# HugoVuach/Dense-linear-app

Hardware: AMD Instinct MI355X
Metric: fp64 TFLOP/s for NxN SPD Cholesky (N^3/3 flops / factorisation time) (higher is better)
Workload: dtype f64

## Files before the change

dense_linear_app_amd/_lib.py:

```python
from __future__ import annotations

import ctypes as C
import os

_HERE = os.path.dirname(os.path.abspath(__file__))
LIB_PATH = os.environ.get("LIBCHOLMI_PATH") or os.path.join(_HERE, "libcholmi.so")

_lib = None


class CholmiError(RuntimeError):

    def __init__(self, fn: str, code: int, msg: str):
        super().__init__(f"{fn} failed with status {code}: {msg}")
        self.fn, self.code, self.msg = fn, code, msg


def lib() -> C.CDLL:
    global _lib
    if _lib is not None:
        return _lib
    if not os.path.exists(LIB_PATH):
        raise ImportError(
            f"{LIB_PATH} is missing: build it with `python -c 'import __graft_entry__ as g; g.build()'` "
# ... 19 lines not shown
        "chol_plgsy_tile": ([d, i, vp, u64], i),
        "chol_lacpy_tile": ([i, vp, vp], i),
        "chol_lange_tile": ([i, vp, C.POINTER(d)], i),
        "chol_lauum_tile": ([i, vp], i),
        "chol_geadd_tile": ([i, d, vp, d, vp], i),
        "chol_potrs_tile": ([i, vp, vp], i),
        "chol_posv_tile": ([i, vp, vp], i),
        "chol_dsposv_tile": ([i, vp, vp, vp, C.POINTER(i)], i),
        "chol_last_dsposv_stats": ([C.POINTER(d)], i),
        "chol_trtri_tile": ([i, i, vp], i),
        "chol_potri_tile": ([i, vp], i),
        "chol_poinv_tile": ([i, vp], i),
        "chol_lansy_tile": ([i, i, vp, C.POINTER(d)], i),
        "chol_pocon_tile": ([i, vp, d, C.POINTER(d)], i),
        "chol_last_pocon_stats": ([C.POINTER(d)], i),
        "chol_poequ_tile": ([vp, vp, C.POINTER(d), C.POINTER(d)], i),
        "chol_laqsy_tile": ([i, vp, vp, d, d, C.POINTER(i)], i),
        "chol_porfs_tile": ([i, vp, vp, vp, vp, C.POINTER(d), C.POINTER(d)], i),
        "chol_posvx_tile": ([i, i, vp, vp, C.POINTER(i), vp, vp, vp, C.POINTER(d), C.POINTER(d), C.POINTER(d)], i),
        "chol_last_posvx_stats": ([C.POINTER(d)], i),
        "chol_bench_refine": ([i, vp, vp, vp, i, i, C.POINTER(d)], i),
        "chol_pstrf_tile": ([i, vp, C.POINTER(i), C.POINTER(i), d], i),
        "chol_last_pstrf_stats": ([C.POINTER(d)], i),
        "chol_sygst_tile": ([i, i, vp, vp], i),
        "chol_last_sygst_stats": ([C.POINTER(d)], i),
        "chol_chud_tile": ([i, vp, vp], i),
        "chol_chdd_tile": ([i, vp, vp], i),
        "chol_last_chud_stats": ([C.POINTER(d)], i),
        "chol_trtrs_tile": ([i, i, i, vp, vp], i),
        "chol_trmm_tile": ([i, i, i, i, d, vp, vp], i),
        "chol_logdet_tile": ([vp, C.POINTER(d)], i),
        "chol_last_trtrs_stats": ([C.POINTER(d)], i),
        "chol_debug_half_limits": ([i, i], i),
        "chol_sytrf_nopiv_tile": ([i, vp], i),
        "chol_sytrs_nopiv_tile": ([i, vp, vp], i),
        "chol_sysv_nopiv_tile": ([i, vp, vp], i),
        "chol_last_sytrf_stats": ([C.POINTER(d)], i),
        "chol_rbt_apply_tile": ([i, vp, vp, i], i),
        "chol_sytrf_rbt_tile": ([i, vp, vp, i, u64], i),
        "chol_sytrs_rbt_tile": ([i, vp, vp, i, vp], i),
        "chol_sysv_rbt_tile": ([i, vp, vp, vp, i, u64, vp, vp, C.POINTER(i), C.POINTER(d)], i),
        "chol_last_rbt_stats": ([C.POINTER(d)], i),
        "chol_lapack_to_tile": ([vp, i, vp], i),
        "chol_tile_to_lapack": ([vp, vp, i], i),
        "chol_tile_upload": ([vp, i, i, vp], i),
        "chol_tile_download": ([vp, i, i, vp], i),
        "chol_residual_plgsy": ([vp, d, u64, C.POINTER(d)], i),
        "chol_residual_plgsy_inf": ([vp, d, u64, C.POINTER(d)], i),
        "chol_make_spd_like_chameleon": ([vp, i, i, d, C.c_char, u64], None),
        "chol_enforce_strict_diag_dominance": ([vp, i, i, d], None),
        "chol_extract_block": ([vp, i, i, i, i, i, vp], None),
        "chol_parse_payloads": ([C.c_char_p, vp, i, vp, vp, vp, vp], i),
        "chol_debug_flow_waves": ([], i),
        "chol_last_potrf_regimes": ([C.POINTER(i), C.POINTER(i)], i),
        "chol_debug_schedule_check": ([i, i, d, d, i, C.c_char_p, i], i),
        "chol_debug_schedule_check_grid": ([i, i, i, i, i, d, d, i, C.c_char_p, i], i),
        "chol_debug_comm_trace": ([i, i, i, i, i, d, d, C.c_char_p, i], i),
        "chol_debug_task_record": ([i, i], i),
        "chol_debug_task_check": ([C.POINTER(C.c_longlong)], i),
        "chol_last_potrf_stats": ([C.POINTER(d), C.POINTER(d), C.POINTER(i), C.POINTER(d)], i),
        "chol_set_profiling": ([i], i),
        "chol_debug_stamps": ([i, C.POINTER(C.c_ulonglong), i], i),
        "chol_mfma_probe": ([i, i, C.POINTER(d)], i),
        "chol_bench_update": ([vp, i, i, i, C.POINTER(d), C.POINTER(d)], i),
        "chol_desc_local_ptr": ([vp, C.POINTER(C.c_size_t)], vp),
        "chol_desc_local_tiles": ([vp, C.POINTER(i), C.POINTER(i)], i),
        "chol_set_transport": ([vp], i),
        "chol_transport_rccl_unique_id": ([vp], i),
        "chol_transport_rccl_init": ([vp, i, i], i),
        "chol_transport_rccl_finalize": ([], i),
        "chol_transport_rccl_version": ([], i),
        "chol_set_transport_channel": ([i, vp], i),
        "chol_transport_selftest": ([i, C.c_size_t], i),
        "chol_set_transport_null": ([], i),
        "chol_dist_rehearse": ([i, i, i, i, i, d, u64, vp, C.POINTER(d)], i),
        "chol_desc_set_version": ([vp, u64], i),
        "chol_tile_batch": ([i, i, i, i, vp, vp, vp, vp, vp, i], i),
        "chol_sync": ([], i),
        "chol_potrf_batch": ([i, i, i, vp, vp, vp, C.POINTER(i), i], i),
        "chol_batch_info": ([i, C.POINTER(i)], i),
        "chol_batch_stats": ([C.POINTER(C.c_longlong)], i),
        "chol_batch_mark": ([C.POINTER(C.c_ulonglong)], i),
        "chol_batch_wait": ([C.POINTER(C.c_ulonglong)], i),
        "chol_debug_calibration": ([C.POINTER(d)], i),
        "chol_debug_update_kernel": ([i, C.c_char_p, i], i),
        "chol_debug_device_counters": ([], i),
        "chol_dist_last_stats": ([C.POINTER(d), C.POINTER(C.c_longlong), C.POINTER(C.c_longlong), C.POINTER(C.c_longlong)], i),
        "chol_dist_factorize_with": ([vp, vp, i, i, i, i, i, i], i),
        "chol_dist_gather_lower": ([vp, vp, i], i),
    }
    for name, (argt, rest) in sig.items():
        try:
            fn = getattr(L, name)
        except AttributeError:
            if os.environ.get("LIBCHOLMI_PATH"):
                continue
            raise
        fn.argtypes = argt
        fn.restype = rest
    _lib = L
    return L


ABI_SYMBOLS = None


# ... 14 lines not shown
```

dense_linear_app_amd/csrc/api.hip:

```cpp
#include <hip/hip_runtime.h>

#include <algorithm>
#include <array>
#include <cmath>
#include <cstdarg>
#include <cstdio>
#include <cstdlib>
#include <cstring>
#include <deque>
#include <mutex>
#include <string>
#include <unordered_map>
#include <vector>

#include "../../include/cholmi.h"
#include "api_internal.h"
#include "cholmi_internal.h"

using namespace cholmi;

extern "C" int chol_internal_walk(chol_desc *d, void *base, cholmi::RankCtx *r, int rank);
extern "C" void chol_internal_dist_finalize(void);
extern "C" int chol_internal_desc_create(chol_desc_t **desc, void *mat, int dtype, int mb, int nb, int bsiz, int lm, int ln,
                                         int i, int j, int m, int n, int p, int q, int my_rank, int nranks);
// ... 789 lines not shown
  }
  for (hipStream_t s : r->retired) (void)hipStreamDestroy(s);
  r->retired.clear();
}

}

extern "C" {

int chol_internal_fail(int code, const char *msg) { return fail(code, msg); }

const char *chol_version(void) { return "cholmi 0.3 (gfx950)"; }

const char *chol_last_error(void) {
  static thread_local std::string copy;
  std::lock_guard<std::mutex> lk(g_err_mu);
  copy = g.last_error;
  return copy.c_str();
}

int chol_set_device(int device) {
  std::lock_guard<std::recursive_mutex> lk(g_mu);
  if (g.inited && device != g.r.device) return fail(-1, "chol_set_device after chol_init");
  g.r.device = device;
  return 0;
}

int chol_set_rank(int rank, int nranks) {
  if (nranks < 1 || rank < 0 || rank >= nranks) return fail(-1, "chol_set_rank: bad rank");
  g.rank = rank;
  g.nranks = nranks;
  return 0;
}

int chol_init(int ncpu, int ngpu) {
  (void)ncpu;
  std::lock_guard<std::recursive_mutex> lk(g_mu);
  if (g.inited) return 0;
  if (ngpu < 1)
    return fail(CHOL_ERR_NO_GPU, "chol_init: ngpu must be >= 1 (this library has no CPU backend)");
  int count = 0;
  hipError_t e = hipGetDeviceCount(&count);
  if (e != hipSuccess || count < 1) {
    (void)hipGetLastError();
    return fail(CHOL_ERR_NO_GPU, "chol_init: no HIP device visible");
  }
  if (g.r.device < 0) {
    const char *lr = getenv("LOCAL_RANK");
    g.r.device = lr ? atoi(lr) % count : 0;
  }
  if (g.r.device >= count) return fail(CHOL_ERR_NO_GPU, "chol_init: device index out of range");
  HIPCHECK(hipSetDevice(g.r.device));
  if (const char *e = getenv("CHOLMI_TRSM_SMALL_MAX")) cholmi::g_trsm_small_max = atoi(e);
  {
    hipDeviceProp_t prop;
    HIPCHECK(hipGetDeviceProperties(&prop, g.r.device));
    const int room = (prop.multiProcessorCount - 32) / 4;
    cholmi::g_poll_max_wgs = room < 0 ? 0 : (room < 48 ? room : 48);
  }
  if (const char *e = getenv("CHOLMI_POLL_MAX_WGS")) cholmi::g_poll_max_wgs = atoi(e);
  if (const char *e = getenv("CHOLMI_FLOW")) cholmi::g_flow = atoi(e);
  if (const char *e = getenv("CHOLMI_FLOW_NBM")) {
    int lo = 0, hi = 0;
    if (sscanf(e, "%d:%d", &lo, &hi) == 2) cholmi::g_flow_min_nbm = std::max(2, lo), cholmi::g_flow_max_nbm = std::min(8, hi);
  }
  if (const char *e = getenv("CHOLMI_FLOW_FENCES")) cholmi::g_flow_fences = atoi(e);
  if (const char *e = getenv("CHOLMI_INTILE_FUSED")) cholmi::g_intile_fused = atoi(e);
  if (const char *e = getenv("CHOLMI_MIN_UNITS")) cholmi::g_min_units = atoi(e);
  HIPCHECK(hipMalloc(&g.d_acc, 2 * sizeof(double)));
  HIPCHECK(hipMalloc(&g.d_ytab, YTAB_ENTRIES * sizeof(int)));
  HIPCHECK(hipMemset(g.d_ytab, 0, YTAB_ENTRIES * sizeof(int)));
  cholmi::g_ytab = g.d_ytab;
  int rc = rank_ctx_create(&g.r, g.r.device, nullptr);
  if (rc) return rc;
  g.inited = true;
  return 0;
}

int chol_finalize(void) {
  std::lock_guard<std::recursive_mutex> lk(g_mu);
  if (!g.inited) return 0;
  (void)hipDeviceSynchronize();
  chol_internal_dist_finalize();
  g.stage.release();
  g.work.release();
  spd_release();
  if (g.wc_winv) (void)hipFree(g.wc_winv);
  g.wc_winv = nullptr;
  if (g.d_binfo) (void)hipFree(g.d_binfo);
  g.d_binfo = nullptr;
  tx_destroy();
  g.wc_ptr = nullptr;
  g.wc_version = 0;
  (void)hipFree(g.d_acc);
  if (g.d_ytab) (void)hipFree(g.d_ytab);
  g.d_ytab = nullptr;
  cholmi::g_ytab = nullptr;
  rank_ctx_destroy(&g.r);
  g.d_acc = nullptr;
  g.inited = false;
  return 0;
}

int chol_desc_create(chol_desc_t **desc, void *mat, int dtype, int mb, int nb, int bsiz, int lm,
                     int ln, int i, int j, int m, int n, int p, int q) {
  return chol_internal_desc_create(desc, mat, dtype, mb, nb, bsiz, lm, ln, i, j, m, n, p, q, g.rank, g.nranks);
// ... 818 lines not shown
    HIPCHECK(hipEventRecord(g.r.events[1], g.r.st[ST_MAIN]));
    HIPCHECK(hipStreamSynchronize(g.r.st[ST_MAIN]));
    float t = 0;
    HIPCHECK(hipEventElapsedTime(&t, g.r.events[0], g.r.events[1]));
    if (r > 0 && t < best) best = t;
  }
  *ms = best;
  const double ntl = (double)(d->nt - 1 - k);
  if (flops) *flops = (ntl * (ntl - 1) + ntl) * (double)d->mbi * d->mbi * d->mbi;
  return 0;
}

int chol_debug_stamps(int enable, unsigned long long *out, int max_pairs) {
  if (!g.inited) return fail(CHOL_ERR_NOT_INITIALIZED, "debug_stamps before chol_init");
  static unsigned long long *buf = nullptr;
  const size_t bytes = (1 + 8 * 1000) * sizeof(unsigned long long);
  HIPCHECK(hipDeviceSynchronize());
  if (enable) {
    if (!buf) HIPCHECK(hipMalloc(&buf, bytes));
    HIPCHECK(hipMemset(buf, 0, bytes));
    cholmi::g_dbg = buf;
    return 0;
  }
  int n = 0;
  if (buf && out) {
    std::vector<unsigned long long> h(1 + 8 * 1000);
    HIPCHECK(hipMemcpy(h.data(), buf, bytes, hipMemcpyDeviceToHost));
    n = (int)std::min<unsigned long long>(h[0], (unsigned long long)std::min(max_pairs, 1000));
    memcpy(out, h.data() + 1, (size_t)n * 8 * sizeof(unsigned long long));
  }
  cholmi::g_dbg = nullptr;
  return n;
}

int chol_mfma_probe(int dtype, int waves_per_simd, double *tflops) {
  if (!g.inited) return fail(CHOL_ERR_NOT_INITIALIZED, "mfma_probe before chol_init");
  if (!tflops || waves_per_simd < 1 || waves_per_simd > 8) return fail(-2, "mfma_probe: arguments");
  std::lock_guard<std::recursive_mutex> lk(g_mu);
  return mfma_probe_on(&g.r, dtype, waves_per_simd, 4000, tflops);
}

int chol_debug_device_counters(void) { return g.inited && g.r.d_sem ? 1 : 0; }

int chol_debug_update_kernel(int dtype, char *buf, int buflen) {
  if (!buf || buflen < 8) return fail(-2, "debug_update_kernel: buffer");
  const bool f64 = dtype == CHOL_REAL_DOUBLE;
  if (!f64 && dtype != CHOL_REAL_FLOAT) return fail(-1, "debug_update_kernel: dtype");
  snprintf(buf, buflen, f64 ? "cholmi::k_trail_update_w8<double, 3>" : "cholmi::k_trail_update_w8f");
  return 0;
}

int chol_debug_flow_waves(void) { return g.r.flow_waves; }

int chol_last_potrf_regimes(int *out8, int *nt) {
  if (!out8) return fail(-1, "last_potrf_regimes: NULL");
  for (int i = 0; i < 8; ++i) out8[i] = g.r.regimes[i];
  if (nt) *nt = g.r.regimes_nt;
  return 0;
}

int chol_debug_calibration(double *out8) {
  if (!g.inited) return fail(CHOL_ERR_NOT_INITIALIZED, "debug_calibration before chol_init");
  if (!out8) return fail(-1, "debug_calibration: NULL");
  for (int i = 0; i < 2; ++i) {
    out8[2 * i] = g.r.probe_tflops[i];
    out8[2 * i + 1] = g.r.diag_us[i];
    out8[4 + 2 * i] = g.r.probe_tflops[i] * CHOLMI_UPDATE_EFF;
    out8[5 + 2 * i] = g.r.diag_us[i] * CHOLMI_STEP_FACTOR;
  }
  return 0;
}

}
```

dense_linear_app_amd/csrc/cholmi_internal.h:

```cpp
#pragma once
#include <hip/hip_runtime.h>
#include <stdint.h>
#include <algorithm>
#include <vector>

#include "../../include/cholmi.h"

struct chol_desc {
  int dtype, mb, nb, bsiz, lm, ln, i, j, m, n, p, q;
  int mbi, bsizi;
  bool padded;
  int mt, nt;
  int prow, pcol;
  int lmt, lnt;
  size_t esize;
  void *mat;
  bool on_device;
  bool owns;
  int2 *d_list = nullptr;
  std::vector<int> ge, gd;
  int n_off = 0;
  unsigned long long version = 0;
  void *user_mat = nullptr;
  int user_lmt = 0;
// ... 31 lines not shown
  }
  void free_all();
};

struct RankCtx {
  int device = -1;
  hipStream_t st[ST_COUNT] = {};
  void *winv = nullptr;
  size_t winv_bytes = 0;
  int *d_info = nullptr;
  int *d_sem = nullptr;
  bool flow_ok = false;
  unsigned tile_sem_next = 0;
  std::vector<hipEvent_t> events;
  std::vector<hipStream_t> retired;
  int stream_swaps = 0;
  int stream_collisions = 0;
  hipEvent_t ev_flow = nullptr;
  bool profiling = false;
  double total_ms = 0, update_ms = 0, update_flops = 0, issue_us = 0;
  int update_launches = 0;
  int flow_waves = 0;
  int regimes[8] = {};
  int regimes_nt = 0;
  long long sends = 0, recvs = 0, bytes_sent = 0;
  DevPool pool;
  double probe_tflops[2] = {0, 0}, diag_us[2] = {0, 0};
};
int rank_ctx_create(RankCtx *r, int device, const RankCtx *calib_from);
void rank_ctx_destroy(RankCtx *r);
RankCtx *main_rank_ctx();
int main_rank(int *nranks);

constexpr double CHOLMI_UPDATE_EFF = 0.85, CHOLMI_STEP_FACTOR = 2.65;

constexpr int MACRO = 128;
constexpr int MAXP = 8;

struct PanelRef {
  const void *base[MAXP];
  int first[MAXP];
  int P;
};

struct LocalMat {
  void *base;
  int lmt;
  int P, Q;
  int mb;
  long bsiz;
};

extern int g_trsm_small_max;
extern int g_poll_max_wgs;
bool flow_applies(int nbm);
extern int g_flow;
extern int g_flow_min_nbm;
extern int g_flow_max_nbm;
extern int g_flow_fences;
extern int g_intile_fused;
extern int g_min_units;
extern unsigned long long *g_dbg;
extern int *g_ytab;
constexpr int YTAB_ENTRIES = 2048;

template <typename T>
void launch_trail_update(hipStream_t s, const LocalMat &C, const int2 *d_list, int off, int na, int offb,
                         int nb, const PanelRef &pan, bool yield = false, const PanelRef *pan2 = nullptr);

template <typename T>
void launch_syr2k_update(hipStream_t s, const LocalMat &C, const int2 *d_list, int off, int na, int offb, int nb,
                         const PanelRef &pan, const PanelRef &qan);

template <typename T>
void launch_ldl_update(hipStream_t s, const LocalMat &C, const int2 *d_list, int off, int na, int offb, int nb,
                       const PanelRef &pan, const PanelRef &qan);

template <typename T>
void launch_potrf_tile(hipStream_t s, T *tile, int mb, T *winv, int *d_info, int info_base, int *sem = nullptr);

template <typename T>
void launch_diag_syrk(hipStream_t s, T *C, const T *A, int mb);

void launch_sem_probe(hipStream_t consumer, hipStream_t producer, int *sem, int *result);
void launch_pipe_probe(hipStream_t big, hipStream_t small, unsigned long long *t, int cus);

struct SyrkPipe {
  void *c;
  hipStream_t su;
  int *sem;
  int *fc = nullptr;
  hipStream_t sflow = nullptr;
  hipEvent_t ev_flow = nullptr;
  bool join_flow = false;
};
inline int flow_ctl_lines(int nbm) { return nbm >= 2 && nbm <= 8 ? 1 + nbm + 2 * nbm * nbm : 0; }

template <typename T>
void launch_panel_pipelined(hipStream_t sp, hipStream_t st, hipEvent_t *ev, T *lkk, int mb, T *winv,
                            int *d_info, int info_base, T *tiles, long bsiz, int ntiles,
                            hipEvent_t ev_head = nullptr, const SyrkPipe *sy = nullptr, const int *wait_sem = nullptr,
                            int wait_target = 0, int *tile_sem = nullptr);

template <typename T>
void launch_col_update_small(hipStream_t s, T *C, const T *A, const T *B, int mb, int ntiles, long bsiz, int *done);

// ... 211 lines not shown
```

dense_linear_app_amd/csrc/kernels.hip:

```cpp
#include "cholmi_internal.h"
#include "mfma_traits.h"

#include <type_traits>

#if defined(__HIP_DEVICE_COMPILE__) && !defined(__gfx950__)
#error "libcholmi's kernels target gfx950 (MI355X) only: build with --offload-arch=gfx950"
#endif

namespace cholmi {

constexpr int BK = 16;
constexpr int LROW = MACRO + 16;

template <int I, int N, typename F>
__device__ __forceinline__ void static_for(F &&f) {
  if constexpr (I < N) {
    f(std::integral_constant<int, I>{});
    static_for<I + 1, N>(f);
  }
}


template <typename T>
struct alignas(16) Smem {
// ... 776 lines not shown
  update_ptr_block<CoreW8<T, MODE>>(cin, ap, bp, cout, n, mb, nbm, unit, ytab, sm);
}
__global__ __launch_bounds__(512, 4) void k_update_ptrs_w8f(const float *const *__restrict__ cin, const float *const *__restrict__ ap,
                                                             const float *const *__restrict__ bp, float *const *__restrict__ cout,
                                                             int n, int mb, int nbm, int unit, const int *ytab) {
  __shared__ SmemF sm;
  update_ptr_block<CoreW8F>(cin, ap, bp, cout, n, mb, nbm, unit, ytab, sm);
}

template <typename T>
__global__ __launch_bounds__(256, 2) void k_panel_solve(T *tiles, long bsiz, int mb, int nbm,
                                                        int s, const T *__restrict__ winv, T alpha,
                                                        int *ytab, const int *wait_sem = nullptr,
                                                        int wait_target = 0, int *fail = nullptr,
                                                        int *head_sem = nullptr) {
  __shared__ SmemP<T> sm;
  sem_wait(wait_sem, wait_target, fail);
  GuestOnCu guest(ytab);
  __builtin_amdgcn_s_setprio(2);
  const int tix = blockIdx.x / nbm, r = blockIdx.x % nbm;
  T *Ap = tiles + (long)tix * bsiz + r * MACRO + (long)s * MACRO * mb;
  const T *Bp = winv + (long)s * MACRO * MACRO;
  Acc<T> acc;
  acc_zero<T>(acc);
  nt_kloop_paired<T>(Ap, mb, Bp, MACRO, MACRO, acc, sm);
  nt_epilogue_paired<T>(Ap, mb, acc, alpha, T(0), false);
  guest.leave();
  if (tix == 0) sem_signal(head_sem);
}

template <typename T>
__global__ __launch_bounds__(256, 2) void k_panel_update(T *tiles, long bsiz, int mb, int nbm, int s,
                                                         const T *__restrict__ lkk, T beta, int *ytab,
                                                         const int *wait_sem = nullptr, int wait_target = 0,
                                                         int *fail = nullptr) {
  __shared__ SmemP<T> sm;
  sem_wait(wait_sem, wait_target, fail);
  GuestOnCu guest(ytab);
  __builtin_amdgcn_s_setprio(2);
  const int nc = nbm - 1 - s;
  int b = blockIdx.x;
  const int c = s + 1 + b % nc;
  b /= nc;
  const int r = b % nbm, tix = b / nbm;
  T *tile = tiles + (long)tix * bsiz;
  const T *Ap = tile + r * MACRO + (long)s * MACRO * mb;
  const T *Bp = lkk + c * MACRO + (long)s * MACRO * mb;
  T *Cp = tile + r * MACRO + (long)c * MACRO * mb;
  Acc<T> acc;
  acc_zero<T>(acc);
  nt_kloop_paired<T>(Ap, mb, Bp, mb, MACRO, acc, sm);
  nt_epilogue_paired<T>(Cp, mb, acc, T(-1), beta, false);
  guest.leave();
}

constexpr int SK = 32;
template <typename T, int ROWS>
struct SmallImg {
  T v[SK][ROWS + 16];
};
template <typename T, int ROWS>
__device__ __forceinline__ void small_gload(const T *__restrict__ P, int ld, int k0, T (&r)[ROWS * SK / 256]) {
#pragma unroll
  for (int q = 0; q < ROWS * SK / 256; ++q) {
    const int e = threadIdx.x + 256 * q;
    r[q] = P[(e % ROWS) + (long)(k0 + e / ROWS) * ld];
  }
}
template <typename T, int ROWS>
__device__ __forceinline__ void small_lstore(SmallImg<T, ROWS> &img, const T (&r)[ROWS * SK / 256]) {
#pragma unroll
  for (int q = 0; q < ROWS * SK / 256; ++q) {
    const int e = threadIdx.x + 256 * q;
    img.v[e / ROWS][e % ROWS] = r[q];
  }
}
template <typename T, int RA, int RB>
__device__ __forceinline__ void small_mma(const SmallImg<T, RA> &ia, const SmallImg<T, RB> &ib, int i0, int j0,
                                          typename Tr<T>::acc_t (&acc)[2][2]) {
  const int lane = threadIdx.x & 63, lo = lane & 15, kq = lane >> 4;
#pragma unroll
  for (int ks = 0; ks < SK / 4; ++ks) {
    const int k = 4 * ks + kq;
    T af[2], bf[2];
#pragma unroll
    for (int a = 0; a < 2; ++a) af[a] = ia.v[k][i0 + 16 * a + lo];
#pragma unroll
    for (int b = 0; b < 2; ++b) bf[b] = ib.v[k][j0 + 16 * b + lo];
#pragma unroll
    for (int a = 0; a < 2; ++a)
#pragma unroll
      for (int b = 0; b < 2; ++b) acc[a][b] = Tr<T>::mfma(bf[b], af[a], acc[a][b]);
  }
}

template <typename T>
__device__ __forceinline__ void small_solve_block(T *Ap, int mb, const T *Bp,
                                                  SmallImg<T, 32> &ia, SmallImg<T, MACRO> &ib) {
  const int lane = threadIdx.x & 63, w = threadIdx.x >> 6, lo = lane & 15;
  T ra[32 * SK / 256], rb[MACRO * SK / 256];
  typename Tr<T>::acc_t acc[2][2];
#pragma unroll
  for (int a = 0; a < 2; ++a)
#pragma unroll
    for (int b = 0; b < 2; ++b)
#pragma unroll
// ... 1135 lines not shown
  __syncthreads();
  for (int c = ty; c < 64; c += 4) {
    ta[tx + (long)c * mb] = sb[tx][c];
    tb[tx + (long)c * mb] = sa[tx][c];
  }
}

template <typename T>
void launch_transpose_inplace(hipStream_t s, T *M, int nt, int mb) {
  const long pairs = (long)nt * (nt + 1) / 2, nsub = mb / 64;
  k_transpose_inplace<T><<<dim3((unsigned)(pairs * nsub * nsub)), 256, 0, s>>>(M, nt, mb);
}
template void launch_transpose_inplace<double>(hipStream_t, double *, int, int);
template void launch_transpose_inplace<float>(hipStream_t, float *, int, int);

template <typename T>
__global__ void k_pad_identity(T *dst, int n, int ldp) {
  const int i = n + blockIdx.x * blockDim.x + threadIdx.x;
  if (i < ldp) dst[i + (size_t)i * ldp] = T(1);
}

__global__ __launch_bounds__(256) void k_pipe_big(unsigned long long *t, int spin_ticks) {
  __shared__ char lds[65536];
  lds[threadIdx.x] = 1;
  const unsigned long long t0 = __builtin_amdgcn_s_memrealtime();
  if (blockIdx.x == 0 && threadIdx.x == 0) t[0] = t0;
  while (__builtin_amdgcn_s_memrealtime() - t0 < (unsigned long long)spin_ticks) __builtin_amdgcn_s_sleep(16);
  if (lds[(threadIdx.x + 1) & 255] == 7) t[2] = 0;
}
__global__ void k_pipe_small(unsigned long long *t) {
  if (threadIdx.x == 0) t[1] = __builtin_amdgcn_s_memrealtime();
}
void launch_pipe_probe(hipStream_t big, hipStream_t small, unsigned long long *t, int cus) {
  k_pipe_big<<<8 * cus, 256, 0, big>>>(t, 2000);
  k_pipe_small<<<1, 64, 0, small>>>(t);
}

void launch_sem_probe(hipStream_t consumer, hipStream_t producer, int *sem, int *result) {
  k_sem_probe_wait<<<1, 1, 0, consumer>>>(sem, result);
  k_sem_probe_set<<<1, 64, 0, producer>>>(sem);
}

int *g_ytab = nullptr;
unsigned long long *g_dbg = nullptr;
int g_min_units = 128;
int g_intile_fused = 1;
constexpr int INTILE_FUSED_MAX = 256;
bool flow_applies(int nbm) { return g_flow && nbm >= g_flow_min_nbm && nbm <= g_flow_max_nbm; }
int g_flow = 1;
int g_flow_min_nbm = 3, g_flow_max_nbm = 4;
int g_flow_fences = 0;
int g_poll_max_wgs = 48;
int g_trsm_small_max = 64;

struct UpdateGrid {
  int unit;
  long blocks_a, blocks_b;
};
inline UpdateGrid update_grid(long tot_a, long tot_b, bool single_diag) {
  UpdateGrid u;
  u.unit = 64;
  while (u.unit > 8 && (tot_a + tot_b) / u.unit < g_min_units) u.unit >>= 1;
  u.blocks_a = ((tot_a + u.unit - 1) / u.unit + 7) / 8 * 8 * u.unit;
  u.blocks_b = ((tot_b + u.unit - 1) / u.unit + 7) / 8 * 8 * u.unit;
  if (single_diag) u.blocks_a = 0, u.blocks_b = tot_b;
  return u;
}

struct UpdateLaunch {
  int offb, nbm, blocks_a, unit;
  dim3 grid;
};
inline UpdateLaunch update_launch(const LocalMat &C, int off, int na, int offb, int nb) {
  const int nbm = C.mb / MACRO, MT = nbm * nbm, MTd = nbm * (nbm + 1) / 2;
  const UpdateGrid u = update_grid((long)na * MT, (long)nb * MTd, na == 0 && nb == 1);
  return {offb - off, nbm, (int)u.blocks_a, u.unit, dim3((unsigned)(u.blocks_a + u.blocks_b))};
}

template <typename T>
void launch_trail_update(hipStream_t s, const LocalMat &C, const int2 *d_list, int off, int na, int offb,
                         int nb, const PanelRef &pan, bool yield, const PanelRef *pan2) {
  if (na + nb <= 0) return;
  const int npan = pan2 ? 2 : 1;
  const PanelRef &p2 = pan2 ? *pan2 : pan;
  const UpdateLaunch l = update_launch(C, off, na, offb, nb);
  if constexpr (sizeof(T) == 4)
    k_trail_update_w8f<<<l.grid, dim3(512), 0, s>>>(C, d_list + off, na, l.offb, nb, l.blocks_a, pan, l.nbm, l.unit,
                                                   yield ? g_ytab : nullptr, p2, npan);
  else
    k_trail_update_w8<T, 3><<<l.grid, dim3(512), 0, s>>>(C, d_list + off, na, l.offb, nb, l.blocks_a, pan, l.nbm, l.unit,
                                                         yield ? g_ytab : nullptr, p2, npan);
}

template <typename T>
void launch_syr2k_update(hipStream_t s, const LocalMat &C, const int2 *d_list, int off, int na, int offb, int nb,
                         const PanelRef &pan, const PanelRef &qan) {
  if (na + nb <= 0) return;
  const UpdateLaunch l = update_launch(C, off, na, offb, nb);
  if constexpr (sizeof(T) == 4)
    k_syr2k_w8f<<<l.grid, dim3(512), 0, s>>>(C, d_list + off, na, l.offb, nb, l.blocks_a, pan, qan, l.nbm, l.unit);
  else
    k_syr2k_w8<T, 3><<<l.grid, dim3(512), 0, s>>>(C, d_list + off, na, l.offb, nb, l.blocks_a, pan, qan, l.nbm, l.unit);
}

template <typename T>
void launch_ldl_update(hipStream_t s, const LocalMat &C, const int2 *d_list, int off, int na, int offb, int nb,
                       const PanelRef &pan, const PanelRef &qan) {
  if (na + nb <= 0) return;
  const UpdateLaunch l = update_launch(C, off, na, offb, nb);
  if constexpr (sizeof(T) == 4)
    k_ldl_update_w8f<<<l.grid, dim3(512), 0, s>>>(C, d_list + off, na, l.offb, nb, l.blocks_a, pan, qan, l.nbm, l.unit);
  else
    k_ldl_update_w8<T, 3><<<l.grid, dim3(512), 0, s>>>(C, d_list + off, na, l.offb, nb, l.blocks_a, pan, qan, l.nbm, l.unit);
}

struct StepSems {
  const int *diag = nullptr;
  const int *intile = nullptr;
  int intile_target = 0;
  int *head = nullptr;
  int *fail = nullptr;
};
template <typename T>
int trsm_step(hipStream_t s, T *tiles, long bsiz, int ntiles, const T *lkk, const T *winv, int mb, int st,
              T alpha, const StepSems &sm = StepSems()) {
  const int nbm = mb / MACRO, nc = nbm - 1 - st;
  if (alpha == T(1) && ntiles * nbm <= g_trsm_small_max) {
    const bool p1 = poll_in_kernel(s, sm.diag, 1, sm.fail, (long)ntiles * nbm * 4);
    k_solve_small<T><<<ntiles * nbm * 4, 256, 0, s>>>(tiles, bsiz, mb, nbm, 0, st, winv, g_ytab,
                                                      p1 ? sm.diag : nullptr, 1, sm.fail, sm.head);
    if (nc > 0) {
      const bool p2 = poll_in_kernel(s, sm.intile, sm.intile_target, sm.fail, 4L * nbm * nc * ntiles);
      k_small_update<T><<<dim3(2 * nbm, 2 * nc, ntiles), 256, 0, s>>>(
          tiles + (long)(st + 1) * MACRO * mb, mb, tiles + (long)st * MACRO * mb,
          lkk + (long)(st + 1) * MACRO + (long)st * MACRO * mb, mb, MACRO, g_ytab, 1, bsiz, bsiz, nullptr,
          p2 ? sm.intile : nullptr, sm.intile_target, sm.fail);
    }
    return 4 * nbm;
  }
  const bool p1 = poll_in_kernel(s, sm.diag, 1, sm.fail, (long)ntiles * nbm);
  k_panel_solve<T><<<ntiles * nbm, 256, 0, s>>>(tiles, bsiz, mb, nbm, st, winv, st == 0 ? alpha : T(1), g_ytab,
                                                p1 ? sm.diag : nullptr, 1, sm.fail, sm.head);
  if (nc > 0) {
    const bool p2 = poll_in_kernel(s, sm.intile, sm.intile_target, sm.fail, (long)ntiles * nbm * nc);
    k_panel_update<T><<<ntiles * nbm * nc, 256, 0, s>>>(tiles, bsiz, mb, nbm, st, lkk, st == 0 ? alpha : T(1), g_ytab,
                                                        p2 ? sm.intile : nullptr, sm.intile_target, sm.fail);
  }
  return nbm;
}

template <typename T>
void launch_col_update_small(hipStream_t s, T *C, const T *A, const T *B, int mb, int ntiles, long bsiz, int *done) {
  if (ntiles > 0) k_small_update<T><<<dim3(mb / 64, mb / 64, ntiles), 256, 0, s>>>(C, mb, A, B, mb, mb, g_ytab, 1, bsiz, bsiz, done);
}
template void launch_col_update_small<double>(hipStream_t, double *, const double *, const double *, int, int, long, int *);
template void launch_col_update_small<float>(hipStream_t, float *, const float *, const float *, int, int, long, int *);

template <typename T>
void launch_diag_syrk(hipStream_t s, T *C, const T *A, int mb) {
  k_small_update<T><<<dim3(mb / 64, mb / 64), 256, 0, s>>>(C, mb, A, A, mb, mb, g_ytab, 0, 0, 0);
}

template <typename T>
void launch_intile_step(hipStream_t stream, T *tile, int mb, int nbm, int s, const T *winv, int *cnt,
                        int *solve_signal, int *d_info) {
  const int nr = nbm - 1 - s;
  if (cnt && nr * (2 * nr + 1) <= INTILE_FUSED_MAX) {
    k_intile_step<T><<<4 * nr + nr * (2 * nr + 1), 256, 0, stream>>>(tile, mb, nbm, s, winv, g_ytab, cnt, d_info);
    return;
  }
  k_solve_small<T><<<4 * nr, 256, 0, stream>>>(tile, 0, mb, nbm, s + 1, s, winv, g_ytab, nullptr, 0, nullptr,
                                               solve_signal);
  T *tr = tile + (long)(s + 1) * MACRO * (mb + 1);
  const T *xs = tile + (long)(s + 1) * MACRO + (long)s * MACRO * mb;
  k_small_update<T><<<dim3(2 * nr, 2 * nr), 256, 0, stream>>>(tr, mb, xs, xs, mb, MACRO, g_ytab, 0, 0, 0);
}

template <typename T>
void launch_potrf_tile(hipStream_t s, T *tile, int mb, T *winv, int *d_info, int info_base, int *sem) {
  const int nbm = mb / MACRO;
  const bool fused_steps = sem && g_intile_fused && nbm > 1;
  if (fused_steps) (void)hipMemsetAsync(sem, 0, (size_t)nbm * 32 * sizeof(int), s);
  for (int st = 0; st < nbm; ++st) {
    k_potrf_diag<T><<<1, 256, 0, s>>>(tile + (long)st * MACRO * (mb + 1), mb,
                                      winv + (long)st * MACRO * MACRO, d_info, info_base + st * MACRO, 1, g_dbg, g_ytab);
    if (st < nbm - 1)
      launch_intile_step<T>(s, tile, mb, nbm, st, winv, fused_steps ? sem + 32 * st : nullptr, nullptr, d_info);
  }
}

template <typename T>
void launch_panel_pipelined(hipStream_t sp, hipStream_t st, hipEvent_t *ev, T *lkk, int mb, T *winv,
                            int *d_info, int info_base, T *tiles, long bsiz, int ntiles, hipEvent_t ev_head,
                            const SyrkPipe *sy, const int *wait_sem, int wait_target, int *tile_sem) {
  const int nbm = mb / MACRO;
  const bool pipe = sy && ntiles > 0;
  const bool fused_plain = !pipe && tile_sem && g_intile_fused && nbm > 1;
  if (fused_plain) (void)hipMemsetAsync(tile_sem, 0, (size_t)nbm * 32 * sizeof(int), sp);
  auto slot = [&](int i) { return sy->sem + 32 * i; };
  const bool flow = pipe && sy->fc && sy->sflow && flow_applies(nbm);
  if (flow) {
    if (sy->join_flow && sy->ev_flow) {
      (void)hipEventRecord(sy->ev_flow, sp);
      (void)hipStreamWaitEvent(sy->sflow, sy->ev_flow, 0);
    }
    k_flow_factor<T><<<nbm, 256, 0, sp>>>(lkk, mb, nbm, winv, d_info, info_base, sy->fc, g_ytab, wait_sem, wait_target,
                                          slot(0), g_flow_fences, g_dbg);
    k_flow_rows<T><<<(mb - MACRO) / 64, 256, 0, sy->sflow>>>(lkk, mb, nbm, winv, d_info, sy->fc, g_ytab, wait_sem, wait_target,
                                                           slot(nbm), g_flow_fences, g_dbg);
  }
  for (int s = 0; s < nbm; ++s) {
    const int nr = nbm - 1 - s;
    if (!flow)
      k_potrf_diag<T><<<1, 256, 0, sp>>>(lkk + (long)s * MACRO * (mb + 1), mb, winv + (long)s * MACRO * MACRO,
                                         d_info, info_base + s * MACRO, 1, g_dbg, g_ytab, s == 0 ? wait_sem : nullptr,
                                         wait_target, pipe ? slot(s) : nullptr);
    if (nr > 0 && !flow) {
      int *const is = pipe ? slot(nbm + s) : nullptr;
      int *const cnt = pipe && g_intile_fused ? is : fused_plain ? tile_sem + 32 * s : nullptr;
      launch_intile_step<T>(sp, lkk, mb, nbm, s, winv, cnt, is, d_info);
    }
    if (ntiles <= 0) continue;
    if (pipe) {
      StepSems ss;
      ss.diag = slot(s);
      ss.intile = slot(nbm + s);
      ss.intile_target = (flow ? 8 : 4) * nr;
      ss.head = sy->c ? slot(2 * nbm + s) : nullptr;
      ss.fail = d_info;
      const int head_wgs = trsm_step<T>(st, tiles, bsiz, ntiles, lkk, winv, mb, s, T(1), ss);
      if (!sy->c) continue;
      const T *xs = tiles + (long)s * MACRO * mb;
      const int n64 = mb / 64;
      const long nslice = (long)n64 * (n64 + 1) / 2;
      int *done = s == nbm - 1 ? slot(3 * nbm) : nullptr;
      const bool ps = poll_in_kernel(sy->su, slot(2 * nbm + s), head_wgs, d_info, nslice);
      k_small_update<T><<<dim3(n64, n64), 256, 0, sy->su>>>(reinterpret_cast<T *>(sy->c), mb, xs, xs, mb, MACRO, g_ytab, 0, 0,
                                                           0, done, ps ? slot(2 * nbm + s) : nullptr, head_wgs, d_info);
      continue;
    }
    (void)hipEventRecord(ev[s], sp);
    (void)hipStreamWaitEvent(st, ev[s], 0);
    trsm_step<T>(st, tiles, bsiz, ntiles, lkk, winv, mb, s, T(1));
  }
  if (ev_head) (void)hipEventRecord(ev_head, st);
}
template void launch_panel_pipelined<double>(hipStream_t, hipStream_t, hipEvent_t *, double *, int, double *,
                                             int *, int, double *, long, int, hipEvent_t, const SyrkPipe *, const int *, int, int *);
template void launch_panel_pipelined<float>(hipStream_t, hipStream_t, hipEvent_t *, float *, int, float *, int *,
                                            int, float *, long, int, hipEvent_t, const SyrkPipe *, const int *, int, int *);

template <typename T>
void launch_invert_diag(hipStream_t s, const T *tile, int mb, T *winv) {
  const int nbm = mb / MACRO;
  for (int st = 0; st < nbm; ++st)
    k_potrf_diag<T><<<1, 256, 0, s>>>(const_cast<T *>(tile) + (long)st * MACRO * (mb + 1), mb,
                                      winv + (long)st * MACRO * MACRO, nullptr, 0, 0, nullptr, g_ytab);
}

template <typename T>
__global__ __launch_bounds__(256, 2) void k_invert_diag_batch(const T *A, long tstride, int mb, T *__restrict__ winv) {
  __shared__ DiagLds<T> L;
  const int nbm = mb / MACRO, t = blockIdx.x / nbm, s = blockIdx.x % nbm;
  potrf_diag_body<T>(const_cast<T *>(A) + t * tstride + (long)s * MACRO * (mb + 1), mb,
                     winv + ((long)t * nbm + s) * MACRO * MACRO, nullptr, 0, 0, L);
}

template <typename T>
void launch_invert_diag_batch(hipStream_t s, const T *A, long tstride, int nt, int mb, T *winv) {
  if (nt > 0) k_invert_diag_batch<T><<<(unsigned)(nt * (mb / MACRO)), 256, 0, s>>>(A, tstride, mb, winv);
}

template <typename T>
void launch_trsm_panel(hipStream_t s, T *tiles, long bsiz, int ntiles, const T *lkk, const T *winv,
                       int mb, T alpha) {
  if (ntiles <= 0) return;
  const int nbm = mb / MACRO;
  for (int st = 0; st < nbm; ++st) trsm_step<T>(s, tiles, bsiz, ntiles, lkk, winv, mb, st, alpha);
}

template <typename T>
void launch_gemm_nt_tile(hipStream_t s, const T *A, const T *B, T *C, int mb, T alpha, T beta,
                         bool lower_only) {
  const int nbm = mb / MACRO;
  k_gemm_nt_tile<T><<<dim3(nbm, nbm), 256, 0, s>>>(A, B, C, mb, nbm, alpha, beta, lower_only ? 1 : 0, 1, 0, 0, 0, 0);
}

template <typename T>
void launch_gemm_nt_batch(hipStream_t s, const T *A, long sA, int nz1, const T *B, long sB, int nz2, T *C, long sC1,
                          long sC2, int mb, T alpha, T beta) {
  const int nbm = mb / MACRO;
  if (nz1 <= 0 || nz2 <= 0) return;
  if (nz1 <= 65535) {
    const int per = std::max(1, 65535 / nz1);
    for (int z2 = 0; z2 < nz2; z2 += per) {
      const int c = std::min(per, nz2 - z2);
      k_gemm_nt_tile<T><<<dim3(nbm, nbm, nz1 * c), 256, 0, s>>>(A, B + (long)z2 * sB, C + (long)z2 * sC2, mb, nbm, alpha, beta, 0,
                                                               nz1, sA, sB, sC1, sC2);
    }
  } else {
    for (int z2 = 0; z2 < nz2; ++z2)
      for (int z1 = 0; z1 < nz1; z1 += 65535) {
        const int c = std::min(65535, nz1 - z1);
        k_gemm_nt_tile<T><<<dim3(nbm, nbm, c), 256, 0, s>>>(A + (long)z1 * sA, B + (long)z2 * sB, C + (long)z1 * sC1 + (long)z2 * sC2,
                                                          mb, nbm, alpha, beta, 0, c, sA, sB, sC1, sC2);
      }
  }
}

template <typename T>
void launch_update_ptrs(hipStream_t s, const T *const *cin, const T *const *a, const T *const *b, T *const *cout, int n, int mb,
                        bool yield) {
  if (n <= 0) return;
  const int nbm = mb / MACRO;
  const UpdateGrid u = update_grid((long)n * nbm * nbm, 0, false);
  const dim3 grid((unsigned)u.blocks_a);
  if constexpr (sizeof(T) == 4)
    k_update_ptrs_w8f<<<grid, dim3(512), 0, s>>>(cin, a, b, cout, n, mb, nbm, u.unit, yield ? g_ytab : nullptr);
  else
    k_update_ptrs_w8<T, 3><<<grid, dim3(512), 0, s>>>(cin, a, b, cout, n, mb, nbm, u.unit, yield ? g_ytab : nullptr);
}
template void launch_update_ptrs<double>(hipStream_t, const double *const *, const double *const *, const double *const *, double *const *, int, int, bool);
template void launch_update_ptrs<float>(hipStream_t, const float *const *, const float *const *, const float *const *, float *const *, int, int, bool);

void launch_copy_ptrs(hipStream_t s, const void *const *src, void *const *dst, int n, long bytes) {
  for (int z0 = 0; z0 < n; z0 += 65535) {
    const int nz = std::min(65535, n - z0);
    k_copy_ptrs<<<dim3((unsigned)std::max(1L, std::min(64L, bytes / (16 * 256 * 4))), nz), 256, 0, s>>>(src + z0, dst + z0, bytes);
  }
}
// ... 76 lines not shown
```

include/cholmi.h:

```cpp
#ifndef CHOLMI_H
#define CHOLMI_H

#include <stddef.h>
#include <stdint.h>

#ifdef __cplusplus
extern "C" {
#endif

enum {
  CHOL_REAL_FLOAT = 2,
  CHOL_REAL_DOUBLE = 3,
  CHOL_NOTRANS = 111,
  CHOL_TRANS = 112,
  CHOL_UPPER = 121,
  CHOL_LOWER = 122,
  CHOL_UPPER_LOWER = 123,
  CHOL_NONUNIT = 131,
  CHOL_UNIT = 132,
  CHOL_LEFT = 141,
  CHOL_RIGHT = 142,
  CHOL_ONE_NORM = 171,
  CHOL_FROBENIUS_NORM = 174,
  CHOL_INF_NORM = 175,
// ... 88 lines not shown

int chol_sygst_tile(int itype, int uplo, chol_desc_t *A, chol_desc_t *B);
int chol_last_sygst_stats(double *out8);

int chol_chud_tile(int uplo, chol_desc_t *A, chol_desc_t *V);
int chol_chdd_tile(int uplo, chol_desc_t *A, chol_desc_t *V);
int chol_last_chud_stats(double *out8);

int chol_trtrs_tile(int uplo, int trans, int diag, chol_desc_t *A, chol_desc_t *B);
int chol_trmm_tile(int side, int uplo, int trans, int diag, double alpha, chol_desc_t *A, chol_desc_t *B);
int chol_logdet_tile(chol_desc_t *A, double *logdet);
int chol_last_trtrs_stats(double *out8);
int chol_debug_half_limits(int trtrs_cols, int trmm_cols);

int chol_sytrf_nopiv_tile(int uplo, chol_desc_t *A);
int chol_sytrs_nopiv_tile(int uplo, chol_desc_t *A, chol_desc_t *B);
int chol_sysv_nopiv_tile(int uplo, chol_desc_t *A, chol_desc_t *B);
int chol_last_sytrf_stats(double *out8);

int chol_rbt_apply_tile(int uplo, chol_desc_t *A, chol_desc_t *W, int depth);
int chol_sytrf_rbt_tile(int uplo, chol_desc_t *A, chol_desc_t *W, int depth, unsigned long long seed);
int chol_sytrs_rbt_tile(int uplo, chol_desc_t *A, chol_desc_t *W, int depth, chol_desc_t *B);
int chol_sysv_rbt_tile(int uplo, chol_desc_t *A, chol_desc_t *AF, chol_desc_t *W, int depth, unsigned long long seed,
                       chol_desc_t *B, chol_desc_t *X, int *iter, double *berr);
int chol_last_rbt_stats(double *out8);

int chol_lapack_to_tile(const void *A, int lda, chol_desc_t *desc);
int chol_tile_to_lapack(chol_desc_t *desc, void *A, int lda);

int chol_tile_upload(chol_desc_t *desc, int I, int J, const void *host_tile);
int chol_tile_download(chol_desc_t *desc, int I, int J, void *host_tile);

int chol_residual_plgsy(chol_desc_t *L, double bump, unsigned long long seed, double *rel);
int chol_residual_plgsy_inf(chol_desc_t *L, double bump, unsigned long long seed, double *rel_inf);

void chol_make_spd_like_chameleon(double *A, int N, int LDA, double bump, char uplo,
                                  unsigned long long seed);
void chol_enforce_strict_diag_dominance(double *A, int N, int LDA, double eps);
int chol_parse_payloads(const char *buf, const long long *off, int n, int *op, int *B, long long *id_off, int *id_len);
void chol_extract_block(const double *A, int N, int LDA, int B, int bi, int bj, double *block);

int chol_last_potrf_stats(double *total_ms, double *update_ms, int *update_launches,
                          double *update_flops);
int chol_last_potrf_regimes(int *out8, int *nt);
int chol_set_profiling(int on);

int chol_bench_update(chol_desc_t *desc, int k, int ablate, int reps, double *ms, double *flops);

int chol_debug_stamps(int enable, unsigned long long *out, int max_pairs);

int chol_mfma_probe(int dtype, int waves_per_simd, double *tflops);

int chol_debug_flow_waves(void);

int chol_debug_schedule_check(int nt, int mb, double t_tile, double t_panel, int profiling, char *report, int cap);
int chol_debug_schedule_check_grid(int nt, int mb, int p, int q, int rank, double t_tile, double t_panel, int profiling,
                                   char *report, int cap);
int chol_debug_comm_trace(int nt, int mb, int p, int q, int rank, double t_tile, double t_panel, char *out, int cap);

int chol_debug_task_record(int on, int mutate);
int chol_debug_task_check(long long *out5);

int chol_debug_calibration(double *out8);
int chol_debug_update_kernel(int dtype, char *buf, int buflen);
int chol_debug_device_counters(void);

void *chol_desc_local_ptr(chol_desc_t *desc, size_t *bytes);
int chol_desc_local_tiles(chol_desc_t *desc, int *lmt, int *lnt);

typedef struct chol_transport {
  void *ctx;
  int (*group_begin)(void *ctx);
  int (*send)(void *ctx, const void *buf, size_t bytes, int peer, void *stream);
  int (*recv)(void *ctx, void *buf, size_t bytes, int peer, void *stream);
  int (*group_end)(void *ctx);
  int (*allreduce_max)(void *ctx, long long *value);
} chol_transport_t;
int chol_set_transport(const chol_transport_t *t);
int chol_set_transport_channel(int channel, const chol_transport_t *t);
#define CHOL_RCCL_ID_BYTES 256
int chol_transport_rccl_unique_id(void *id256);
int chol_transport_rccl_init(const void *id256, int rank, int nranks);
int chol_transport_rccl_finalize(void);
int chol_transport_rccl_version(void);
int chol_dist_last_stats(double *issue_us_per_wave, long long *sends, long long *recvs, long long *bytes_sent);

int chol_dist_gather_lower(chol_desc_t *src, chol_desc_t *dst, int root);

int chol_set_transport_null(void);

int chol_transport_selftest(int self_rank, size_t bytes);

typedef struct chol_test_engine {
  void *ctx;
  void *store;
  size_t esize;
  void *(*alloc)(void *ctx, size_t bytes);
  int (*potrf)(void *ctx, int k, void *lkk);
  int (*trsm)(void *ctx, int k, const void *lkk);
  int (*update)(void *ctx, int k, int jlo, int jhi, const void *const *bases, const int *firsts, int skip_diag);
  int (*update_diag)(void *ctx, int k, int j, const void *const *bases, const int *firsts);
  int (*info)(void *ctx);
} chol_test_engine_t;
int chol_dist_factorize_with(const chol_test_engine_t *engine, const chol_transport_t *transport, int N, int B,
                             int p, int q, int rank, int mode);

// ... 8 lines not shown
```

Before: 70.54.

## Add left-looking panel TRSM path for large tile panels

Adds a left-looking variant of the blocked panel triangular solve. For each macro column it first applies all previously solved columns in a single MFMA GEMM kernel (k-depth MACRO*c), then runs the diagonal block solve. This replaces the right-looking sequence of per-step trailing updates with one accumulate-then-store pass per column, cutting repeated reads and writes of the panel. It is used only when the panel has enough blocks and alpha is one. The trade-off is that the GEMM depth grows with the column index, and very small panels keep the old path.

```diff
diff --git a/dense_linear_app_amd/_lib.py b/dense_linear_app_amd/_lib.py
--- a/dense_linear_app_amd/_lib.py
+++ b/dense_linear_app_amd/_lib.py
@@ -95,6 +95,7 @@
         "chol_extract_block": ([vp, i, i, i, i, i, vp], None),
         "chol_parse_payloads": ([C.c_char_p, vp, i, vp, vp, vp, vp], i),
         "chol_debug_flow_waves": ([], i),
+        "chol_debug_trsm_left_steps": ([], C.c_longlong),
         "chol_last_potrf_regimes": ([C.POINTER(i), C.POINTER(i)], i),
         "chol_debug_schedule_check": ([i, i, d, d, i, C.c_char_p, i], i),
         "chol_debug_schedule_check_grid": ([i, i, i, i, i, d, d, i, C.c_char_p, i], i),
diff --git a/dense_linear_app_amd/csrc/api.hip b/dense_linear_app_amd/csrc/api.hip
--- a/dense_linear_app_amd/csrc/api.hip
+++ b/dense_linear_app_amd/csrc/api.hip
@@ -865,6 +865,8 @@
   if (g.r.device >= count) return fail(CHOL_ERR_NO_GPU, "chol_init: device index out of range");
   HIPCHECK(hipSetDevice(g.r.device));
   if (const char *e = getenv("CHOLMI_TRSM_SMALL_MAX")) cholmi::g_trsm_small_max = atoi(e);
+  if (const char *e = getenv("CHOLMI_TRSM_LEFT_MIN")) cholmi::g_trsm_left_min = atoi(e);
+  cholmi::g_trsm_left_steps = 0;
   {
     hipDeviceProp_t prop;
     HIPCHECK(hipGetDeviceProperties(&prop, g.r.device));
@@ -1789,6 +1791,8 @@
 
 int chol_debug_flow_waves(void) { return g.r.flow_waves; }
 
+long long chol_debug_trsm_left_steps(void) { return cholmi::g_trsm_left_steps; }
+
 int chol_last_potrf_regimes(int *out8, int *nt) {
   if (!out8) return fail(-1, "last_potrf_regimes: NULL");
   for (int i = 0; i < 8; ++i) out8[i] = g.r.regimes[i];
diff --git a/dense_linear_app_amd/csrc/cholmi_internal.h b/dense_linear_app_amd/csrc/cholmi_internal.h
--- a/dense_linear_app_amd/csrc/cholmi_internal.h
+++ b/dense_linear_app_amd/csrc/cholmi_internal.h
@@ -107,6 +107,8 @@
 };
 
 extern int g_trsm_small_max;
+extern int g_trsm_left_min;
+extern long long g_trsm_left_steps;
 extern int g_poll_max_wgs;
 bool flow_applies(int nbm);
 extern int g_flow;
diff --git a/dense_linear_app_amd/csrc/kernels.hip b/dense_linear_app_amd/csrc/kernels.hip
--- a/dense_linear_app_amd/csrc/kernels.hip
+++ b/dense_linear_app_amd/csrc/kernels.hip
@@ -852,6 +852,35 @@
   nt_kloop_paired<T>(Ap, mb, Bp, mb, MACRO, acc, sm);
   nt_epilogue_paired<T>(Cp, mb, acc, T(-1), beta, false);
   guest.leave();
+}
+
+template <typename Core>
+__device__ __forceinline__ void panel_left_block(typename Core::T *tiles, long bsiz, int mb, int nbm, int c,
+                                                 const typename Core::T *lkk, typename Core::Smem &sm) {
+  using T = typename Core::T;
+  const int tix = blockIdx.x / nbm, r = blockIdx.x % nbm;
+  T *tile = tiles + (long)tix * bsiz;
+  T *Cp = tile + r * MACRO + (long)c * MACRO * mb;
+  typename Core::Acc acc;
+#pragma unroll
+  for (int a = 0; a < 4; ++a)
+#pragma unroll
+    for (int b = 0; b < 2; ++b)
+#pragma unroll
+      for (int q = 0; q < 4; ++q) acc[a][b][q] = T(0);
+  Core::kloop(tile + r * MACRO, mb, lkk + c * MACRO, mb, MACRO * c, acc, sm, nullptr);
+  Core::template epilogue<false>(Cp, Cp, mb, acc, false);
+}
+template <typename T, int MODE>
+__global__ __launch_bounds__(512, 4) void k_panel_left_w8(T *tiles, long bsiz, int mb, int nbm, int c,
+                                                           const T *__restrict__ lkk) {
+  __shared__ SmemR<T> sm;
+  panel_left_block<CoreW8<T, MODE>>(tiles, bsiz, mb, nbm, c, lkk, sm);
+}
+__global__ __launch_bounds__(512, 4) void k_panel_left_w8f(float *tiles, long bsiz, int mb, int nbm, int c,
+                                                            const float *__restrict__ lkk) {
+  __shared__ SmemF sm;
+  panel_left_block<CoreW8F>(tiles, bsiz, mb, nbm, c, lkk, sm);
 }
 
 constexpr int SK = 32;
@@ -2093,6 +2122,8 @@
 int g_flow_fences = 0;
 int g_poll_max_wgs = 48;
 int g_trsm_small_max = 64;
+int g_trsm_left_min = 304;
+long long g_trsm_left_steps = 0;
 
 struct UpdateGrid {
   int unit;
@@ -2188,6 +2219,24 @@
                                                         p2 ? sm.intile : nullptr, sm.intile_target, sm.fail);
   }
   return nbm;
+}
+
+bool trsm_left_applies(int ntiles, int mb, bool alpha_is_one) {
+  const int nbm = mb / MACRO;
+  const long blocks = (long)ntiles * nbm;
+  return alpha_is_one && mb % MACRO == 0 && nbm >= 2 && blocks > g_trsm_small_max && blocks >= g_trsm_left_min;
+}
+template <typename T>
+void trsm_left_step(hipStream_t s, T *tiles, long bsiz, int ntiles, const T *lkk, const T *winv, int mb, int c) {
+  const int nbm = mb / MACRO;
+  if (c > 0) {
+    if constexpr (sizeof(T) == 4)
+      k_panel_left_w8f<<<ntiles * nbm, 512, 0, s>>>(tiles, bsiz, mb, nbm, c, lkk);
+    else
+      k_panel_left_w8<T, 3><<<ntiles * nbm, 512, 0, s>>>(tiles, bsiz, mb, nbm, c, lkk);
+  }
+  k_panel_solve<T><<<ntiles * nbm, 256, 0, s>>>(tiles, bsiz, mb, nbm, c, winv, T(1), g_ytab);
+  ++g_trsm_left_steps;
 }
 
 template <typename T>
@@ -2282,7 +2331,10 @@
     }
     (void)hipEventRecord(ev[s], sp);
     (void)hipStreamWaitEvent(st, ev[s], 0);
-    trsm_step<T>(st, tiles, bsiz, ntiles, lkk, winv, mb, s, T(1));
+    if (trsm_left_applies(ntiles, mb, true))
+      trsm_left_step<T>(st, tiles, bsiz, ntiles, lkk, winv, mb, s);
+    else
+      trsm_step<T>(st, tiles, bsiz, ntiles, lkk, winv, mb, s, T(1));
   }
   if (ev_head) (void)hipEventRecord(ev_head, st);
 }
@@ -2317,6 +2369,10 @@
                        int mb, T alpha) {
   if (ntiles <= 0) return;
   const int nbm = mb / MACRO;
+  if (trsm_left_applies(ntiles, mb, alpha == T(1))) {
+    for (int st = 0; st < nbm; ++st) trsm_left_step<T>(s, tiles, bsiz, ntiles, lkk, winv, mb, st);
+    return;
+  }
   for (int st = 0; st < nbm; ++st) trsm_step<T>(s, tiles, bsiz, ntiles, lkk, winv, mb, st, alpha);
 }
 
diff --git a/include/cholmi.h b/include/cholmi.h
--- a/include/cholmi.h
+++ b/include/cholmi.h
@@ -164,6 +164,7 @@
 int chol_mfma_probe(int dtype, int waves_per_simd, double *tflops);
 
 int chol_debug_flow_waves(void);
+long long chol_debug_trsm_left_steps(void);
 
 int chol_debug_schedule_check(int nt, int mb, double t_tile, double t_panel, int profiling, char *report, int cap);
 int chol_debug_schedule_check_grid(int nt, int mb, int p, int q, int rank, double t_tile, double t_panel, int profiling,
```

New measurement: 70.84 (median of 6 runs). No clear change (+0.4%).
